# 14chanwa/remotesensingProject

Measured on AMD Instinct MI355X. Metric: Mpixel*disparity-hypotheses/s, higher is better.
Workload: dtype f32

## Files before the change

include/rslf_hip.h:

```cpp
#ifndef RSLF_HIP_H
#define RSLF_HIP_H

#include <stddef.h>
#include <stdint.h>

#ifdef __cplusplus
extern "C" {
#endif

#define RSLF_ABI_VERSION 6

typedef enum rslf_status {
    RSLF_OK = 0,
    RSLF_ERR_INVALID_ARG = -1,
    RSLF_ERR_UNSUPPORTED = -2,
    RSLF_ERR_HIP = -3,
    RSLF_ERR_NO_DEVICE = -4,
    RSLF_ERR_ALLOC = -5,
    RSLF_ERR_INTERNAL = -6
} rslf_status;

typedef struct rslf_params {
    float edge_score_threshold;
    float line_score_threshold;
// ... 327 lines not shown
int rslf_render_fit(rslf_ctx* ctx, const float* d_plane, int rows, int cols, size_t row_stride, const uint8_t* d_valid, int mode,
                    double* h_min, double* h_max);
int rslf_render_fit_many(rslf_ctx* ctx, const float* d_planes, int n_planes, size_t plane_stride, int rows, int cols, size_t row_stride,
                         const uint8_t* d_valid, int mode, double* h_minmax);
int rslf_render_planes(rslf_ctx* ctx, const float* d_planes, int n_planes, size_t plane_stride, int rows, int cols, size_t row_stride,
                       double min, double max, int formula, const uint8_t* lut_bgr, const uint8_t* d_valid, int mask_mode,
                       const rslf_volume* vol, int slice_kind, int index, float shadow_level, uint8_t* d_bgr_out);
int rslf_render_planes_each(rslf_ctx* ctx, const float* d_planes, int n_planes, size_t plane_stride, int rows, int cols, size_t row_stride,
                            const double* h_minmax, int formula, const uint8_t* lut_bgr, const uint8_t* d_valid, int mask_mode,
                            const rslf_volume* vol, int slice_kind, int index, float shadow_level, uint8_t* d_bgr_out);
int rslf_render_planes_host(rslf_ctx* ctx, const float* h_planes, int n_planes, size_t plane_stride, int rows, int cols, size_t row_stride,
                            const uint8_t* h_valid, int fit_mode, int fit_plane, int fit_masked, int formula, const uint8_t* lut_bgr,
                            int mask_mode, const rslf_volume* vol, int slice_kind, int index, float shadow_level, uint8_t* h_bgr_out,
                            double* h_minmax);
int rslf_render_epi_lines(rslf_ctx* ctx, const float* d_depth_vu, const uint8_t* d_mask_vu, int V, int S, int U, int s_hat, int v_first,
                          int n_rows, const uint8_t* lut_bgr, uint8_t* d_bgr_out);
int rslf_render_epi_lines_host(rslf_ctx* ctx, const float* h_depth_vu, const uint8_t* h_mask_vu, int V, int S, int U, int s_hat, int v_first,
                               int n_rows, const uint8_t* lut_bgr, uint8_t* h_bgr_out);
int rslf_render_centre_index(int n, int* index);
int rslf_render_scaled_row(int v, int dim_v, int dim_v_orig, int* row);

int rslf_last_scan_kernel_ms(rslf_ctx* ctx, float* ms);
int rslf_scan_time_total_ms(rslf_ctx* ctx, float* ms, int* launches);

#ifdef __cplusplus
}
#endif
#endif
```

remotesensingproject_amd/_lib.py:

```python
from __future__ import annotations

import ctypes as C
import os

from . import build as _build

_LIB = None

ABI_VERSION = 6

SYMBOLS = [
    "rslf_abi_version", "rslf_status_string", "rslf_last_error", "rslf_device_count", "rslf_default_params",
    "rslf_ctx_create", "rslf_ctx_destroy", "rslf_ctx_set_stream", "rslf_ctx_synchronize", "rslf_ctx_set_debug", "rslf_debug_inject",
    "rslf_multi_create", "rslf_multi_destroy", "rslf_multi_device_count", "rslf_multi_set_chunk_rows", "rslf_multi_peer_access",
    "rslf_multi_depth1d_pile_f32", "rslf_multi_depth1d_pile_u8", "rslf_multi_depth1d_pile_f32_dev",
    "rslf_multi_depth2d_run_f32", "rslf_multi_depth2d_run_u8", "rslf_multi_fine_to_coarse_run_host",
    "rslf_volume_create", "rslf_volume_destroy", "rslf_volume_describe",
    "rslf_volume_upload_epis_f32", "rslf_volume_upload_epis_u8",
    "rslf_volume_upload_images_f32", "rslf_volume_upload_images_u8", "rslf_volume_pack_device_f32",
    "rslf_edge_confidence_pile", "rslf_depth_epi_pile", "rslf_selective_median",
    "rslf_depth1d_pile_run", "rslf_depth1d_pile_run_host", "rslf_last_scan_kernel_ms", "rslf_scan_time_total_ms",
    "rslf_edge_confidence_2d", "rslf_depth_epi_2d", "rslf_depth2d_run",
    "rslf_sweep_begin", "rslf_sweep_visit_scan", "rslf_sweep_visit_finish", "rslf_sweep_end",
    "rslf_depth_epi_scan", "rslf_depth1d_run",
    "rslf_f2c_level_dims", "rslf_downsample_epis_f32", "rslf_downsample_epis_u8", "rslf_device_max_f32", "rslf_f2c_tighten_bounds", "rslf_f2c_fuse",
    "rslf_depth2d_run_host", "rslf_fine_to_coarse_run_host", "rslf_kernel_columns_pile", "rslf_volume_upload_images_xf_f32", "rslf_volume_upload_images_xf_u8",
    "rslf_volume_upload_epis_u16", "rslf_volume_upload_images_u16", "rslf_volume_upload_images_xf_u16", "rslf_downsample_epis_u16",
    "rslf_multi_depth1d_pile_u16", "rslf_multi_depth2d_run_u16", "rslf_fine_to_coarse_run_host_u16",
    "rslf_multi_fine_to_coarse_run_host_u16",
    "rslf_render_fit", "rslf_render_planes", "rslf_render_epi_lines", "rslf_render_centre_index", "rslf_render_scaled_row",
    "rslf_render_fit_many", "rslf_render_planes_each", "rslf_render_planes_host", "rslf_render_epi_lines_host",
    "rslf_line_confidence_pile", "rslf_sweep_line_confidence", "rslf_depth_epi_2d_lc", "rslf_depth2d_run_lc", "rslf_depth2d_run_host_lc",
    "rslf_f2c_pyramid_dims", "rslf_fine_to_coarse_run_host_lc", "rslf_fine_to_coarse_run_host_u16_lc",
    "rslf_f2c_run_host", "rslf_f2c_run_destroy", "rslf_f2c_run_describe", "rslf_f2c_run_copy", "rslf_f2c_run_volume",
    "rslf_f2c_run_render_depth_maps", "rslf_f2c_run_render_depth_maps_host", "rslf_f2c_run_render_depth_pyr",
    "rslf_f2c_run_render_depth_pyr_host", "rslf_f2c_run_render_epi_pyr", "rslf_f2c_run_render_epi_pyr_host",
    "rslf_depth_epi_scores", "rslf_depth_epi_scores_host",
]


class RslfParams(C.Structure):

    _fields_ = [
        ("edge_score_threshold", C.c_float),
# ... 108 lines not shown
    L.rslf_volume_upload_images_f32.argtypes = [vp, C.POINTER(vp), C.c_size_t, cf, C.POINTER(cf)]
    L.rslf_volume_upload_images_u8.argtypes = [vp, C.POINTER(vp), C.c_size_t]
    L.rslf_volume_upload_images_xf_f32.argtypes = [vp, C.POINTER(vp), C.c_size_t, cf, C.POINTER(cf), ci, ci]
    L.rslf_volume_upload_images_xf_u8.argtypes = [vp, C.POINTER(vp), C.c_size_t, ci, ci]
    L.rslf_volume_upload_epis_u16.argtypes = L.rslf_volume_upload_epis_f32.argtypes
    L.rslf_volume_upload_images_u16.argtypes = L.rslf_volume_upload_images_f32.argtypes
    L.rslf_volume_upload_images_xf_u16.argtypes = L.rslf_volume_upload_images_xf_f32.argtypes
    L.rslf_volume_pack_device_f32.argtypes = [vp, vp, cf, C.POINTER(cf)]
    L.rslf_edge_confidence_pile.argtypes = [vp, vp, ci, C.POINTER(RslfParams), vp, vp]
    L.rslf_depth_epi_pile.argtypes = [vp, vp, vp, vp, cf, cf, ci, ci, vp, vp, vp, vp, vp, C.POINTER(RslfParams),
                                      vp, vp, vp, vp, C.POINTER(RslfStats)]
    L.rslf_selective_median.argtypes = [vp, vp, vp, vp, ci, ci, vp, cf]
    L.rslf_depth_epi_scan.argtypes = [vp, vp, vp, vp, cf, cf, ci, ci, vp, vp, vp, vp, vp, C.POINTER(RslfParams),
                                      vp, vp, vp, C.POINTER(RslfStats)]
    L.rslf_depth_epi_scores.argtypes = [vp, vp, vp, vp, cf, cf, ci, ci, C.POINTER(RslfParams), vp, ci, ci, vp, C.POINTER(RslfStats)]
    L.rslf_depth_epi_scores_host.argtypes = L.rslf_depth_epi_scores.argtypes
    L.rslf_depth1d_run.argtypes = [vp, vp, cf, cf, ci, ci, C.POINTER(RslfParams), vp, vp, vp, vp, vp, vp, vp,
                                   C.POINTER(RslfStats)]
    L.rslf_depth1d_pile_run.argtypes = [vp, vp, cf, cf, ci, ci, C.POINTER(RslfParams), vp, vp, vp, vp, vp, vp, vp, vp,
                                        C.POINTER(RslfStats)]
    L.rslf_depth1d_pile_run_host.argtypes = L.rslf_depth1d_pile_run.argtypes
    L.rslf_last_scan_kernel_ms.argtypes = [vp, C.POINTER(cf)]
    L.rslf_scan_time_total_ms.argtypes = [vp, C.POINTER(cf), C.POINTER(ci)]
    L.rslf_sweep_begin.argtypes = [vp, vp, vp, vp, ci, ci, ci]
    L.rslf_sweep_visit_scan.argtypes = [vp, vp, vp, vp, cf, cf, ci, ci, vp, vp, vp, vp, vp, C.POINTER(RslfParams)]
    L.rslf_sweep_visit_finish.argtypes = [vp, vp, ci, vp, vp, vp, vp, C.POINTER(RslfParams)]
    L.rslf_sweep_end.argtypes = [vp, ci, ci, C.POINTER(RslfStats)]
    L.rslf_multi_create.argtypes = [C.POINTER(ci), ci, C.POINTER(vp)]
    L.rslf_multi_destroy.argtypes = [vp]
    L.rslf_multi_device_count.argtypes = [vp]
    L.rslf_multi_set_chunk_rows.argtypes = [vp, ci]
    L.rslf_multi_peer_access.argtypes = [vp, ci, ci]
    L.rslf_debug_inject.argtypes = [C.c_char_p, ci]
    L.rslf_multi_depth1d_pile_f32.argtypes = [vp, C.POINTER(vp), C.c_size_t, ci, ci, ci, ci, cf, cf, cf, ci, ci, C.POINTER(RslfParams),
                                              vp, vp, vp, vp, vp, vp, vp, vp, C.POINTER(RslfStats), C.POINTER(cf)]
    L.rslf_multi_depth1d_pile_f32_dev.argtypes = [vp, C.POINTER(vp), C.c_size_t, ci, ci, ci, ci, cf, cf, cf, ci, ci, C.POINTER(RslfParams), ci,
                                                  vp, vp, vp, vp, vp, vp, vp, vp, C.POINTER(RslfStats), C.POINTER(cf)]
    L.rslf_multi_depth1d_pile_u8.argtypes = [vp, C.POINTER(vp), C.c_size_t, ci, ci, ci, ci, cf, cf, ci, ci, C.POINTER(RslfParams),
                                             vp, vp, vp, vp, vp, vp, vp, vp, C.POINTER(RslfStats)]
    L.rslf_multi_depth2d_run_f32.argtypes = [vp, C.POINTER(vp), C.c_size_t, ci, ci, ci, ci, cf, cf, cf, ci, C.POINTER(RslfParams),
                                             vp, vp, vp, vp, vp, vp, C.POINTER(RslfStats), C.POINTER(cf)]
    L.rslf_multi_depth1d_pile_u16.argtypes = L.rslf_multi_depth1d_pile_f32.argtypes
    L.rslf_multi_depth2d_run_u16.argtypes = L.rslf_multi_depth2d_run_f32.argtypes
    L.rslf_multi_depth2d_run_u8.argtypes = [vp, C.POINTER(vp), C.c_size_t, ci, ci, ci, ci, cf, cf, ci, C.POINTER(RslfParams),
                                            vp, vp, vp, vp, vp, vp, C.POINTER(RslfStats)]
    L.rslf_multi_fine_to_coarse_run_host.argtypes = [vp, C.POINTER(vp), ci, ci, ci, ci, ci, C.c_size_t, cf, cf, ci, cf, C.POINTER(RslfParams),
# ... 68 lines not shown
```

remotesensingproject_amd/csrc/k2_reg.hpp:

```cpp
#pragma once

#include "k2_scan.hpp"
#include "k2_taps.hpp"

namespace rslf {

#ifndef RSLF_REG_GB104
#define RSLF_REG_GB104 8
#endif
constexpr int gather_batch(int c) { return c == 1 ? 8 : 4; }
constexpr int kPadSlack = 16;

template <int SPAD, int C, bool PK, bool KONLY>
__device__ __forceinline__ void mean_shift_pass(const float (&R)[PK ? 1 : C][PK ? 1 : SPAD], const f2 (&R2)[PK ? C : 1][PK ? SPAD / 2 : 1],
                                                int S, float kq, const float (&rbar)[C], float (&A)[C], float& B)
{
    static_assert(!KONLY || (C == 1 && !PK), "the K-only pass is written for the scalar one-channel blocks");
    if constexpr (PK) {
        f2 rb2[C];
        const f2 kq2 = {kq, kq};
#pragma unroll
        for (int c = 0; c < C; c++)
            rb2[c] = f2{rbar[c], rbar[c]};
        constexpr int kBlk = (C == 1) ? 8 : 4;
// ... 456 lines not shown
#ifndef RSLF_REG_BEST_LDS
#define RSLF_REG_BEST_LDS 1
#endif
constexpr bool scan_reg_best_in_lds(int spad, int c)
{
    if (!RSLF_REG_BEST_LDS)
        return false;
    if (c == 1)
        return spad == 16 || spad == 40 || spad == 48 || (spad >= 80 && spad <= 88) || (spad >= 104 && spad <= 144);
    return spad == 24 || spad == 40;
}

constexpr bool scan_reg_packed_math(int spad, int c) { return scan_reg_waves(spad, c) == 1; }

constexpr bool scan_reg_trim(int spad, int c)
{
    return c == 1 && !scan_reg_packed_math(spad, c) && spad != 48 && !(spad >= 80 && spad <= 88) && !(spad > 112 && spad <= 144);
}
#ifndef RSLF_TAP_TABLE
#define RSLF_TAP_TABLE 1
#endif
constexpr bool scan_reg_tap_table(int spad, int c) { return RSLF_TAP_TABLE && c == 1 && spad == 104 && scan_reg_trim(spad, c); }

template <int SPAD, int C>
using ScanRegRbarFix = std::conditional_t<scan_reg_trim(SPAD, C), LastPassRbar<C>, NoRbarFix>;

template <int SPAD, int C, class BestT>
__device__ __forceinline__ void scan_reg_rows(const ScanArgs& a, int v, int u, int d0, int d1, BestT& best, float* otab)
{
    constexpr bool PK = scan_reg_packed_math(SPAD, C);
    constexpr bool kTaps = scan_reg_tap_table(SPAD, C);
    if (a.dmin_vu) {
        scan_reg_body<SPAD, C, true, false, PK, 0, BestT, false, scan_reg_trim(SPAD, C)>(a, v, u, d0, d1, best, otab);
        return;
    }
    const float max_ds = (float)max(a.s_hat, a.vol.S - 1 - a.s_hat);
    const float range = a.dmax - a.dmin, denom = (float)(a.dim_d - 1);
    const float uf = (float)u, Um1 = (float)(a.vol.U - 1);
    auto interior = [&](int d) -> bool {
        const float reach = max_ds * fabsf(hypothesis(a.dmin, range, denom, d)) * fabsf(a.k.slope) + 2.0f;
        return __all((uf - reach >= 0.0f) && (uf + reach <= Um1));
    };
    int d = d0;
    while (d < d1) {
        const bool in = interior(d);
        int e = d + 1;
        while (e < d1 && interior(e) == in)
            e++;
        if (in)
            scan_reg_body<SPAD, C, false, true, PK, 0, BestT, false, scan_reg_trim(SPAD, C), kTaps>(a, v, u, d, e, best, otab);
        else
            scan_reg_body<SPAD, C, true, true, PK, 0, BestT, false, scan_reg_trim(SPAD, C)>(a, v, u, d, e, best, otab);
        d = e;
    }
}

template <int SPAD, int C>
__global__ __launch_bounds__(64 * kScanWaves) __attribute__((amdgpu_waves_per_eu(scan_reg_waves(SPAD, C), scan_reg_waves(SPAD, C))))
void k2_scan_reg(ScanArgs a)
{
    __shared__ __attribute__((aligned(16))) float s_otab[kScanWaves][SPAD * (scan_reg_tap_table(SPAD, C) ? 4 : 1)];
// ... 72 lines not shown
```

remotesensingproject_amd/csrc/k2_scan.hpp:

```cpp
#pragma once

#include <type_traits>

#include "rslf_device.hpp"

namespace rslf {

constexpr int kScanWaves = 4;
#ifndef RSLF_XCD_ROW_INTERLEAVE
#define RSLF_XCD_ROW_INTERLEAVE 1
#endif

struct ScanArgs {
    VolView vol;
    const int* list;
    const int* count;
    const float* dmin_vu;
    const float* dmax_vu;
    float dmin, dmax;
    int dim_d, s_hat;
    ScanConsts k;
    float* Ce;
    uint8_t* Ce_mask;
    float* Cd;
    float* depth;
    float* rbar;
    int32_t* idx;
    float* score;
    int tile_w;
    int tiles_per_row;
    int logical_blocks;
    int per_xcd;
    int groups;
    struct Partial* partial;
    int* ticket;
    int v0;
    int packed;
    const int* packed_n;
    int packed_adapt;
    int stream_park;
    int stream_wave_floats;
    float stream_frac_max;
    int px_waves;
    const int* rowbase;
    int row_min;
    int tap_table;
};

struct Partial {
    float score, D;
    int d;
    float rbar[3];
    double sum;
};

template <int C>
struct Best {
    float score;
    int d;
    float D;
    float rbar[C];
    double sum;
    __device__ __forceinline__ void init()
    {
        score = -1.0f;
        d = 0;
        D = 0.0f;
#pragma unroll
        for (int c = 0; c < C; c++)
            rbar[c] = 0.0f;
// ... 549 lines not shown
```

remotesensingproject_amd/csrc/k2_taps.hpp:

```cpp
#pragma once

#include <math.h>
#include <stdint.h>
#include <string.h>

#if defined(__HIPCC__)
#define RSLF_TAPS_FN __host__ __device__ __forceinline__
#else
#define RSLF_TAPS_FN inline
#endif

namespace rslf {

struct TapEntry {
    int byteoff;
    float t, omt;
    bool fast;
};

RSLF_TAPS_FN uint32_t tap_float_bits(float x)
{
#if defined(__HIP_DEVICE_COMPILE__)
    return __float_as_uint(x);
#else
// ... 20 lines not shown
#else
    return (int)floorf(x);
#endif
}

RSLF_TAPS_FN TapEntry tap_entry(float off, int u_first, int u_last, int U, int C, int row_floats)
{
    const float uf = (float)u_first, ul = (float)u_last;
    const float x_first = off + uf;
    const float x_last = off + ul;
    TapEntry e;
    e.t = tap_fract(x_first);
    const int i0 = tap_floor(x_first);
    e.omt = 1.0f - e.t;
    e.byteoff = (int)((unsigned)(i0 * C + row_floats) << 2);
    const bool inside = x_first > 0.0f && x_last <= (float)(U - 1);
    const bool binade = ((tap_float_bits(x_first) ^ tap_float_bits(x_last)) >> 23) == 0;
    const float back = x_last - ul;
    const bool exact = back == off;
    e.fast = inside && (binade || exact);
    return e;
}

}
```

remotesensingproject_amd/csrc/rslf_core.hip:

```cpp
#include "rslf_internal.hpp"

#include <algorithm>
#include <cmath>

#include "k0_pack.hpp"

using namespace rslf;


namespace rslf {

char* last_error_buffer()
{
    static thread_local char g_err[512] = "";
    return g_err;
}

static std::atomic<int> g_inject[kInjectSites];

bool inject_hit(InjectSite site)
{
    std::atomic<int>& c = g_inject[site];
    int v = c.load(std::memory_order_relaxed);
    while (v > 0)
// ... 194 lines not shown
    ctx->stream = (hipStream_t)hip_stream;
    return RSLF_OK;
}
RSLF_API_CATCH

extern "C" int rslf_ctx_set_debug(rslf_ctx* ctx, const char* key, int value) RSLF_API_TRY
{
    if (!ctx || !key)
        return fail(RSLF_ERR_INVALID_ARG, "ctx/key is NULL");
    if (strcmp(key, "force_scan") == 0 && value >= 0 && value <= 2)
        ctx->force_scan = value;
    else if (strcmp(key, "force_groups") == 0 && value >= 0 && value <= 64)
        ctx->force_groups = value;
    else if (strcmp(key, "force_packed") == 0 && value >= -1 && value <= 1)
        ctx->force_packed = value;
    else if (strcmp(key, "px") == 0 && value >= -1 && value <= 1)
        ctx->px_mode = value;
    else if (strcmp(key, "stream_share") == 0 && value >= 0 && value <= 2)
        ctx->stream_share = value;
    else if (strcmp(key, "row_split") == 0 && value >= 0 && value <= 65536)
        ctx->row_split = value;
    else if (strcmp(key, "tap_table") == 0 && (value == 0 || value == 1))
        ctx->tap_table = value;
    else if (strcmp(key, "claim_skip") == 0 && (value == 0 || value == 1))
        ctx->claim_skip = value;
    else if (strcmp(key, "time_all") == 0 && (value == 0 || value == 1)) {
        ctx->time_all = value;
        ctx->ev_used = 0;
    } else if (strcmp(key, "stream_groups") == 0 && value >= 0 && value <= 64)
        ctx->stream_groups = value;
    else if (strcmp(key, "stream_lds_kib") == 0 && value >= 16 && value <= 152) {
        ctx->stream_lds_bytes = (size_t)value << 10;
    } else if (strcmp(key, "staging_kib") == 0 && value >= 0 && value <= 262144)
        ctx->staging_kib = value;
    else
        return fail(RSLF_ERR_INVALID_ARG, "rslf_ctx_set_debug: unknown key or value out of range: %s = %d", key, value);
    return RSLF_OK;
}
RSLF_API_CATCH

extern "C" int rslf_ctx_synchronize(rslf_ctx* ctx) RSLF_API_TRY
{
    if (!ctx)
        return fail(RSLF_ERR_INVALID_ARG, "ctx is NULL");
    HIP_TRY(hipSetDevice(ctx->device));
    HIP_TRY(hipStreamSynchronize(ctx->stream));
// ... 484 lines not shown
```

remotesensingproject_amd/csrc/rslf_internal.hpp:

```cpp
#pragma once

#include "../../include/rslf_hip.h"

#include <hip/hip_runtime.h>

#include <atomic>
#include <cstdarg>
#include <cstdio>
#include <cstring>
#include <exception>
#include <functional>
#include <memory>
#include <new>
#include <string>
#include <thread>
#include <vector>

#include "rslf_device.hpp"
#include "rslf_plan.hpp"
#include "rslf_scratch.hpp"


namespace rslf {

// ... 112 lines not shown
enum SharedBuf {
    kSharedLevel = 0,
    kSharedTable,
    kSharedLeft,
    kSharedRight,
    kSharedStagePlanes,
    kSharedStageMask,
    kSharedStageOut,
    kSharedBufs
};

struct Scratch {
    DeviceBuf total;
    DeviceBuf minmax;
    DeviceBuf list;
    DeviceBuf depth_tmp;
    DeviceBuf count;
    DeviceBuf rowbase;
    DeviceBuf partial;
    DeviceBuf staging;
    DeviceBuf scan_partial;
    DeviceBuf scan_ticket;
    DeviceBuf max_partial;
    DeviceBuf winner;
    DeviceBuf sweep_mask;
    DeviceBuf dirty;
    DeviceBuf remain;
    DeviceBuf filtered;
    DeviceBuf lc_columns;
    DeviceBuf lc_argmax;
    DeviceBuf shared[kSharedBufs];

    static constexpr size_t kMaxPartials = 2048;
    unsigned long long* pixel_total() const { return total.as<unsigned long long>(); }
    int* packed_len() const { return reinterpret_cast<int*>(pixel_total() + 1); }
    uint8_t* morph_tmp() const { return depth_tmp.as<uint8_t>(); }
};

struct SweepState {
    bool open = false;
    bool keep_total = false;
    bool first = true;
    bool scanned = false;
    bool listed = false;
    int expect = -1;
    uint8_t* mask_run = nullptr;
    int lc_mode = RSLF_LINE_CONF_OFF;
    float* lc_Cl_svu = nullptr;
    float* lc_K_vsu = nullptr;
    int32_t* lc_idx_vu = nullptr;
    const float* lc_Ce_svu = nullptr;
    const float* lc_dmin_vu = nullptr;
    const float* lc_dmax_vu = nullptr;
    float lc_dmin = 0.0f, lc_dmax = 0.0f;
    int lc_dim_d = 0;
    ScanConsts lc_consts = {};
};

}

struct rslf_ctx {
    int device = 0;
    hipStream_t stream = nullptr;
    rslf::Scratch scratch;
    rslf::SweepState sweep;
    hipEvent_t ev0 = nullptr, ev1 = nullptr;
    bool ev_valid = false;
    int time_all = 0;
    std::vector<hipEvent_t> ev_pool;
    size_t ev_used = 0;
    int last_spad = 0;
    int last_kernel = 0;
    int num_cus = 0;
    int force_scan = 0;
    int force_groups = 0;
    int force_packed = -1;
    int px_mode = -1;
    int stream_groups = 0;
    int stream_share = 1;
    size_t stream_lds_bytes = rslf::plan::kStreamLdsBytes;
    int row_split = 1;
    int tap_table = 1;
    int claim_skip = 1;
    int staging_kib = 0;
};

struct rslf_volume {
    rslf_ctx* ctx = nullptr;
    int device = 0;
    int V = 0, S = 0, U = 0, C = 0, pitch = 0;
    float* base = nullptr;
    size_t bytes = 0;
    float min_value = 0.0f, max_value = 0.0f;
    bool filled = false;
};

struct rslf_multi {
    struct Dev {
        rslf_ctx* ctx = nullptr;
        hipStream_t s_up = nullptr, s_comp = nullptr, s_down = nullptr;
        hipEvent_t done[2] = {nullptr, nullptr};
        rslf_volume* vol[2] = {nullptr, nullptr};
        rslf::DeviceBuf planes[2];
        rslf::PinnedBuf pin[2];
        rslf::DeviceBuf arena;
// ... 143 lines not shown
```

remotesensingproject_amd/csrc/rslf_pile.hip:

```cpp
#include "rslf_internal.hpp"

#include <algorithm>
#include <cmath>

#include "k1_edge.hpp"
#include "k2_scan.hpp"
#include "k2_reg.hpp"
#include "k2_stream.hpp"
#include "k3_median.hpp"

using namespace rslf;

static_assert(sizeof(Partial) == plan::kPartialRecordBytes, "rslf_plan.hpp sizes the record scratch");
static_assert(kScanWaves == plan::kScanWavesPerTile, "rslf_plan.hpp shares the hypotheses out over this many waves");


extern "C" int rslf_edge_confidence_pile(rslf_ctx* ctx, const rslf_volume* vol, int s, const rslf_params* p,
                                         float* d_Ce_vu, uint8_t* d_Ce_mask_vu) RSLF_API_TRY
{
    if (!ctx || !vol || !d_Ce_vu || !d_Ce_mask_vu)
        return fail(RSLF_ERR_INVALID_ARG, "NULL argument");
    int rc = check_params(p);
    if (rc)
        return rc;
    if (s < 0 || s >= vol->S)
        return fail(RSLF_ERR_INVALID_ARG, "s=%d outside [0,%d)", s, vol->S);
    if (!vol->filled)
        return fail(RSLF_ERR_INVALID_ARG, "volume has not been filled");
    HIP_TRY(hipSetDevice(ctx->device));
    EdgeConsts ec;
    ec.filter_size = p->edge_confidence_filter_size;
    ec.cut_shadows = p->cut_shadows;
    ec.shadow_level = p->shadow_level;
    ec.edge_thr = p->edge_score_threshold;
    const dim3 grid((vol->U + 255) / 256, vol->V);
    if (vol->C == 1)
        hipLaunchKernelGGL(k1_edge_confidence<1>, grid, dim3(256), 0, ctx->stream, view_of(vol), s, ec, d_Ce_vu, d_Ce_mask_vu);
// ... 121 lines not shown
{
    const int spad = plan::pick_spad(S, C);
    return plan::ScanKernelFacts{spad ? scan_reg_waves(spad, C) : 0, stream_resident_for(S, C), stream_px_resident_for(S, C)};
}

static plan::ScanRequest scan_request(const rslf_ctx* ctx, int V, int U, int S, int C, int dim_d, bool in_range, bool linear,
                                      bool pixel_ranges, const ScanInputs& in)
{
    plan::ScanRequest rq = {};
    rq.V = V, rq.U = U, rq.S = S, rq.C = C, rq.dim_d = dim_d;
    rq.num_cus = ctx->num_cus;
    rq.ctx_groups = in.groups;
    rq.ctx_packed = in.packed;
    rq.precompacted = in.lists;
    rq.force_groups = ctx->force_groups;
    rq.force_packed = ctx->force_packed;
    rq.px_mode = ctx->px_mode;
    rq.stream_groups = ctx->stream_groups;
    rq.stream_share = ctx->stream_share;
    rq.stream_lds_bytes = ctx->stream_lds_bytes;
    rq.tap_table = ctx->tap_table;
    const bool dense_uniform = !pixel_ranges && !in.packed && ctx->force_packed != 1 && in.lists != ScanInputs::kPackedList;
    plan::choose_scan_kernel(&rq, in_range, linear, ctx->force_scan, dense_uniform, kernel_facts(S, C));
    return rq;
}

int rslf::scan_presize(rslf_ctx* ctx, int S, int U, int C, int dim_d, const rslf_params* p, const int* rows, int n_rows)
{
    const plan::ScanKernelFacts f = kernel_facts(S, C);
    int max_rows = 0;
    size_t recs = 0, tickets = 0;
    for (int i = 0; i < n_rows; i++) {
        max_rows = std::max(max_rows, rows[i]);
        ScanInputs in;
        if (p && plan::fuse_k1_compaction(p->edge_confidence_opening_size, ctx->force_packed, (size_t)rows[i] * U))
            in.lists = ScanInputs::kRowLists;
        const plan::ScanRequest rq = scan_request(ctx, rows[i], U, S, C, dim_d, true, !p || p->interpolation == RSLF_INTERP_LINEAR, false, in);
        const plan::ScanPlan sp = plan::plan_scan(rq, f.nres, f.nres_px);
        recs = std::max(recs, sp.records);
        tickets = std::max(tickets, sp.tickets);
    }
    if (max_rows < 1)
        return RSLF_OK;
    HIP_TRY(hipSetDevice(ctx->device));
    bool tickets_fresh = false;
    int rc = ensure_plane_scratch(ctx, max_rows, U);
// ... 32 lines not shown

ScanInputs rslf::scan_defaults(const rslf_ctx* ctx)
{
    ScanInputs in;
    in.zero_total = !ctx->sweep.keep_total;
    in.timed = !ctx->sweep.open || ctx->sweep.first;
    return in;
}

static int check_scan_args(const rslf_volume* vol, const float* d_dmin_vu, const float* d_dmax_vu, int dim_d, int s_hat,
                           const rslf_params* p)
{
    int rc = check_params(p);
    if (rc)
        return rc;
    if ((d_dmin_vu == nullptr) != (d_dmax_vu == nullptr))
        return fail(RSLF_ERR_INVALID_ARG, "d_dmin_vu and d_dmax_vu must both be given or both be NULL");
    if (dim_d < 2)
        return fail(RSLF_ERR_INVALID_ARG, "dim_d=%d: the hypothesis grid divides by dim_d-1 (core.hpp:548)", dim_d);
    if (s_hat < 0 || s_hat >= vol->S)
        return fail(RSLF_ERR_INVALID_ARG, "s_hat=%d outside [0,%d)", s_hat, vol->S);
    if (!vol->filled)
        return fail(RSLF_ERR_INVALID_ARG, "volume has not been filled");
    return RSLF_OK;
}

static void apply_plan(ScanArgs& a, const plan::ScanPlan& p, const rslf_ctx* ctx)
{
    a.groups = p.groups;
    a.tile_w = p.tile_w;
    a.tiles_per_row = p.tiles_per_row;
    a.packed = p.packed ? 1 : 0;
    a.packed_adapt = p.packed_adapt ? 1 : 0;
    a.px_waves = p.px_waves;
    a.tap_table = p.tap_table;
    a.stream_park = p.stream_park;
    a.stream_wave_floats = p.stream_wave_floats;
    a.partial = p.groups > 1 ? ctx->scratch.scan_partial.as<Partial>() : nullptr;
    a.ticket = p.groups > 1 ? ctx->scratch.scan_ticket.as<int>() : nullptr;
}

static int enqueue_scan(const plan::ScanPlan& p, const ScanArgs& a, unsigned grid_x, size_t stream_lds_bytes, hipStream_t st)
{
    const dim3 grid(grid_x), block(64 * kScanWaves);
    const int C = a.vol.C;
    hipError_t attr = hipSuccess;
// ... 98 lines not shown
    a.list = sc.list.as<int>();
    a.count = sc.count.as<int>();
    a.dmin_vu = d_dmin_vu;
    a.dmax_vu = d_dmax_vu;
    a.dmin = dmin;
    a.dmax = dmax;
    a.dim_d = dim_d;
    a.s_hat = s_hat;
    a.k = make_scan_consts(p);
    a.Ce = d_Ce_vu;
    a.Ce_mask = d_Ce_mask_vu;
    a.Cd = d_Cd_vu;
    a.depth = d_depth_vu;
    a.rbar = d_rbar_vu;
    a.idx = d_idx_vu;
    a.score = d_score_vu;
    a.stream_frac_max = plan::stream_frac_max(vol->U);
    a.packed_n = packed_n;
    a.row_min = row_min;
    ScanArgs ar = a;
    apply_plan(a, sp, ctx);
    apply_plan(ar, spr, ctx);
    ar.rowbase = sc.rowbase.as<int>();
    ctx->last_spad = sp.spad;
    ctx->last_kernel = sp.kind;
    HIP_TRY(hipGetLastError());

    const bool pooled = ctx->time_all && ctx->ev_used + 2 <= ((size_t)1 << 16);
    while (pooled && ctx->ev_pool.size() < ctx->ev_used + 2) {
        hipEvent_t e = nullptr;
        HIP_TRY(hipEventCreate(&e));
        ctx->ev_pool.push_back(e);
    }
    auto enqueue_all = [&]() -> int {
        if (pooled)
            HIP_TRY(hipEventRecord(ctx->ev_pool[ctx->ev_used - 2], st));
        if (in.timed)
            HIP_TRY(hipEventRecord(ctx->ev0, st));
        for (const plan::ScanLaunch& l : row_launches) {
            ar.v0 = l.v0, ar.logical_blocks = l.logical_blocks, ar.per_xcd = l.per_xcd;
            if (int e = enqueue_scan(spr, ar, l.grid, ctx->stream_lds_bytes, st))
                return e;
        }
        for (const plan::ScanLaunch& l : launches) {
            a.v0 = l.v0, a.logical_blocks = l.logical_blocks, a.per_xcd = l.per_xcd;
            if (int e = enqueue_scan(sp, a, l.grid, ctx->stream_lds_bytes, st))
// ... 212 lines not shown
}
RSLF_API_CATCH

extern "C" int rslf_scan_time_total_ms(rslf_ctx* ctx, float* ms, int* launches) RSLF_API_TRY
{
    if (!ctx || !ms)
        return fail(RSLF_ERR_INVALID_ARG, "NULL argument");
    HIP_TRY(hipSetDevice(ctx->device));
    double sum = 0.0;
    for (size_t i = 0; i + 1 < ctx->ev_used; i += 2) {
        float t = 0.0f;
        HIP_TRY(hipEventSynchronize(ctx->ev_pool[i + 1]));
        HIP_TRY(hipEventElapsedTime(&t, ctx->ev_pool[i], ctx->ev_pool[i + 1]));
        sum += (double)t;
    }
    *ms = (float)sum;
    if (launches)
        *launches = (int)(ctx->ev_used / 2);
    ctx->ev_used = 0;
    return RSLF_OK;
}
RSLF_API_CATCH

extern "C" int rslf_last_scan_kernel_ms(rslf_ctx* ctx, float* ms) RSLF_API_TRY
{
    if (!ctx || !ms)
        return fail(RSLF_ERR_INVALID_ARG, "NULL argument");
    if (!ctx->ev_valid)
        return fail(RSLF_ERR_INVALID_ARG, "no scan kernel has been launched on this context");
    HIP_TRY(hipSetDevice(ctx->device));
    HIP_TRY(hipEventSynchronize(ctx->ev1));
    HIP_TRY(hipEventElapsedTime(ms, ctx->ev0, ctx->ev1));
    return RSLF_OK;
}
RSLF_API_CATCH
```

remotesensingproject_amd/csrc/rslf_plan.hpp:

```cpp
#pragma once

#include <stddef.h>
#include <stdint.h>

#include <string.h>

#include <algorithm>
#include <cmath>
#include <vector>

#include "../../include/rslf_hip.h"

namespace rslf {

struct MorphElement {
    int k;
    unsigned rows[31];
};

namespace plan {


constexpr int kScanWavesPerTile = 4;
constexpr size_t kPartialRecordBytes = 32;
// ... 556 lines not shown
            best = w;
        }
    }
    return best_use >= 0.6 ? best : 0;
}

struct ScanRequest {
    int V, U, S, C, dim_d;
    int spad;
    bool use_stream;
    bool use_chip;
    int chip_wave_floats;
    int reg_waves;
    int num_cus;
    int ctx_groups;
    bool ctx_packed;
    int precompacted;
    int force_groups;
    int force_packed;
    int px_mode;
    int stream_groups;
    int stream_share;
    size_t stream_lds_bytes;
    int tap_table;
};

struct ScanPlan {
    int kind;
    int spad;
    int groups;
    bool packed;
    bool packed_adapt;
    int px_waves;
    int tap_table;
    int tile_w;
    int tiles_per_row;
    int rows_per_launch;
    size_t records;
    size_t tickets;
    int stream_nres;
    int stream_park;
    int stream_wave_floats;
    size_t lds_bytes;
};

inline int stream_resident_hi(int C, int nres_1ch, int nres_rgb) { return C == 1 ? nres_1ch : nres_rgb; }

struct ScanKernelFacts {
    int reg_waves;
    int nres;
    int nres_px;
};

inline bool scan_range_ok(float min_value, float max_value) { return min_value >= 0.0f && max_value <= 1.0e6f; }

inline void choose_scan_kernel(ScanRequest* r, bool in_range, bool linear, int force_scan, bool dense_uniform, const ScanKernelFacts& f)
{
// ... 61 lines not shown
    if (packed && (r.spad || r.use_stream) && !r.use_chip && r.px_mode != 0) {
        px_w = px_waves(r.dim_d);
        if (px_w == 0 && r.px_mode == 1)
            px_w = 1;
    }
    if (px_w && r.use_stream && nres_px >= 0)
        nres = nres_px;
    p.stream_nres = r.use_stream ? nres : 0;
    const int park_early = r.use_stream ? stream_park_for(r.S, r.C, nres, r.stream_lds_bytes) : 0;
    const bool share = r.use_chip ? r.stream_share != 0
                                  : r.use_stream && (r.stream_share == 2 || (r.stream_share == 1 && stream_shares_taps(r.S, nres, park_early)));
    p.tile_w = (share && !packed) ? 63 : 64;
    p.tiles_per_row = p.tile_w == 63 ? std::max(1, (r.U + 61) / 63) : (r.U + p.tile_w - 1) / p.tile_w;
    p.packed_adapt = packed && !r.use_stream && !r.use_chip;
    p.rows_per_launch = r.V;
    if (groups > 1 && !packed) {
        const size_t per_row = (size_t)p.tiles_per_row * groups * 64 * kPartialRecordBytes;
        p.rows_per_launch = (int)std::min<size_t>((size_t)r.V, std::max<size_t>(1, kPartialBudget / per_row));
    }
    if (packed && (r.use_stream || r.use_chip))
        while (groups > 1 && ((n + 63) / 64) * groups * 64 * kPartialRecordBytes > kPartialBudget)
            groups /= 2;
    p.px_waves = px_w;
    p.tap_table = (r.spad && !packed && r.tap_table) ? 1 : 0;
    p.spad = r.spad;
    p.kind = r.spad ? (px_w ? RSLF_SCAN_REG_PX : RSLF_SCAN_REG)
             : r.use_chip ? RSLF_SCAN_CHIP
             : r.use_stream ? (px_w ? RSLF_SCAN_STREAM_PX : RSLF_SCAN_STREAM) : RSLF_SCAN_GENERIC;
    if (px_w) {
        groups = 1;
        p.packed_adapt = false;
    }
    p.groups = groups;
    p.packed = packed;
    p.records = 0;
    p.tickets = 0;
    if (groups > 1) {
        const size_t tiles_all = (n + 63) / 64;
        const size_t tiles_max = !packed ? (size_t)p.rows_per_launch * p.tiles_per_row
                                         : p.packed_adapt ? std::min<size_t>(tiles_all, kPackedItemTarget / 2) : tiles_all;
        p.records = (packed && p.packed_adapt) ? std::min<size_t>(tiles_all * groups, kPackedItemTarget) * 64 : tiles_max * groups * 64;
        p.tickets = tiles_max;
    }
    p.stream_park = 0;
    p.stream_wave_floats = 0;
    p.lds_bytes = 0;
    if (r.use_stream) {
// ... 261 lines not shown
```

remotesensingproject_amd/depth.py:

```python
from __future__ import annotations

import atexit
import copy
import ctypes as C
import sys
from dataclasses import dataclass
from typing import Optional, Sequence

import numpy as np
import torch

from . import _lib
from ._lib import RslfParams, RslfStats, RslfVolumeDesc, check


class Interpolation1DLinear:
    mode = 0


class Interpolation1DNearestNeighbour:

    def __init__(self, as_built: bool = False):
        self.mode = 2 if as_built else 1

# ... 43 lines not shown
        raise ValueError("%s: par_line_confidence_mode=%d is not built here (one-device Depth2DComputer only)"
                         % (who, int(parameters.par_line_confidence_mode)))


class Context:

    def __init__(self, device: int | torch.device | None = None):
        if device is None:
            device = torch.cuda.current_device()
        self.device = torch.device("cuda", device) if isinstance(device, int) else torch.device(device)
        h = C.c_void_p()
        check(_lib.lib().rslf_ctx_create(self.device.index or 0, C.byref(h)), "rslf_ctx_create")
        self._h = h
        self.use_current_stream()

    def use_current_stream(self) -> None:
        s = torch.cuda.current_stream(self.device).cuda_stream
        check(_lib.lib().rslf_ctx_set_stream(self._h, C.c_void_p(s)), "rslf_ctx_set_stream")

    def synchronize(self) -> None:
        check(_lib.lib().rslf_ctx_synchronize(self._h), "rslf_ctx_synchronize")

    _DEBUG_DEFAULTS = dict(force_scan=0, force_groups=0, force_packed=-1, px=-1, stream_share=1, stream_groups=0, stream_lds_kib=80,
                           claim_skip=1, time_all=0, row_split=1, staging_kib=0, tap_table=1)
    _FORCE_SCAN = {None: 0, "auto": 0, "generic": 1, "stream": 2}

    def set_debug(self, **hooks) -> None:
        for k, v in hooks.items():
            if k == "force_scan" and not isinstance(v, int):
                v = self._FORCE_SCAN[v or None]
            check(_lib.lib().rslf_ctx_set_debug(self._h, k.encode(), int(v)), "rslf_ctx_set_debug(%s)" % k)

    def reset_debug(self) -> None:
        self.set_debug(**self._DEBUG_DEFAULTS)

    def last_scan_kernel_ms(self) -> float:
        ms = C.c_float()
        check(_lib.lib().rslf_last_scan_kernel_ms(self._h, C.byref(ms)), "rslf_last_scan_kernel_ms")
        return float(ms.value)

    def scan_time_total_ms(self) -> tuple[float, int]:
        ms, n = C.c_float(), C.c_int()
        check(_lib.lib().rslf_scan_time_total_ms(self._h, C.byref(ms), C.byref(n)), "rslf_scan_time_total_ms")
        return float(ms.value), int(n.value)

    def close(self) -> None:
        if getattr(self, "_h", None) and not sys.is_finalizing():
            _lib.lib().rslf_ctx_destroy(self._h)
        self._h = None

    def __del__(self):
        try:
            self.close()
        except Exception:
            pass


_DEFAULT_CTX: dict[int, Context] = {}


@atexit.register
def _drop_default_contexts() -> None:
# ... 1104 lines not shown
```

Before: 8353.

## Precompute per-hypothesis row tap offsets and weights for scalar-load register scan

```diff
diff --git a/include/rslf_hip.h b/include/rslf_hip.h
--- a/include/rslf_hip.h
+++ b/include/rslf_hip.h
@@ -373,6 +373,7 @@
 
 int rslf_last_scan_kernel_ms(rslf_ctx* ctx, float* ms);
 int rslf_scan_time_total_ms(rslf_ctx* ctx, float* ms, int* launches);
+int rslf_last_scan_row_exact(rslf_ctx* ctx, int* attached, int* exact_hypotheses);
 
 #ifdef __cplusplus
 }
diff --git a/remotesensingproject_amd/_lib.py b/remotesensingproject_amd/_lib.py
--- a/remotesensingproject_amd/_lib.py
+++ b/remotesensingproject_amd/_lib.py
@@ -19,7 +19,7 @@
     "rslf_volume_upload_epis_f32", "rslf_volume_upload_epis_u8",
     "rslf_volume_upload_images_f32", "rslf_volume_upload_images_u8", "rslf_volume_pack_device_f32",
     "rslf_edge_confidence_pile", "rslf_depth_epi_pile", "rslf_selective_median",
-    "rslf_depth1d_pile_run", "rslf_depth1d_pile_run_host", "rslf_last_scan_kernel_ms", "rslf_scan_time_total_ms",
+    "rslf_depth1d_pile_run", "rslf_depth1d_pile_run_host", "rslf_last_scan_kernel_ms", "rslf_scan_time_total_ms", "rslf_last_scan_row_exact",
     "rslf_edge_confidence_2d", "rslf_depth_epi_2d", "rslf_depth2d_run",
     "rslf_sweep_begin", "rslf_sweep_visit_scan", "rslf_sweep_visit_finish", "rslf_sweep_end",
     "rslf_depth_epi_scan", "rslf_depth1d_run",
@@ -174,6 +174,7 @@
     L.rslf_depth1d_pile_run_host.argtypes = L.rslf_depth1d_pile_run.argtypes
     L.rslf_last_scan_kernel_ms.argtypes = [vp, C.POINTER(cf)]
     L.rslf_scan_time_total_ms.argtypes = [vp, C.POINTER(cf), C.POINTER(ci)]
+    L.rslf_last_scan_row_exact.argtypes = [vp, C.POINTER(ci), C.POINTER(ci)]
     L.rslf_sweep_begin.argtypes = [vp, vp, vp, vp, ci, ci, ci]
     L.rslf_sweep_visit_scan.argtypes = [vp, vp, vp, vp, cf, cf, ci, ci, vp, vp, vp, vp, vp, C.POINTER(RslfParams)]
     L.rslf_sweep_visit_finish.argtypes = [vp, vp, ci, vp, vp, vp, vp, C.POINTER(RslfParams)]
diff --git a/remotesensingproject_amd/csrc/k2_reg.hpp b/remotesensingproject_amd/csrc/k2_reg.hpp
--- a/remotesensingproject_amd/csrc/k2_reg.hpp
+++ b/remotesensingproject_amd/csrc/k2_reg.hpp
@@ -502,6 +502,102 @@
 #endif
 constexpr bool scan_reg_tap_table(int spad, int c) { return RSLF_TAP_TABLE && c == 1 && spad == 104 && scan_reg_trim(spad, c); }
 
+#ifndef RSLF_SCALAR_TAPS
+#define RSLF_SCALAR_TAPS 1
+#endif
+#ifndef RSLF_SCALAR_GB
+#define RSLF_SCALAR_GB 13
+#endif
+constexpr bool scan_reg_scalar_taps(int spad, int c) { return RSLF_SCALAR_TAPS && scan_reg_tap_table(spad, c); }
+
+template <int SPAD, class BestT>
+__device__ __forceinline__ void scan_reg_body_scalar(const ScanArgs& a, int v, int u, int d0, int d1, BestT& best)
+{
+    constexpr int C = 1, BATCH = RSLF_SCALAR_GB, ROUNDS = SPAD / BATCH;
+    static_assert(SPAD % BATCH == 0, "whole rounds");
+    static_assert(!scan_reg_packed_math(SPAD, 1) && scan_reg_trim(SPAD, 1), "the passes below are the scalar TRIM ones of the other forms");
+    typedef const __attribute__((address_space(4))) long long* OffPtr;
+    typedef const __attribute__((address_space(4))) f2* WeightPtr;
+    typedef const __attribute__((address_space(4))) float* FloatPtr;
+    const VolView& vol = a.vol;
+    const float* epi = vol.row(v, 0);
+    const int S = vol.S;
+    const float kq = a.k.k1;
+    const unsigned ubytes = (unsigned)u << 2;
+    const float centre = epi[(long long)a.s_hat * vol.stride_s + u];
+    const f2 R2[1][1] = {{f2{0.0f, 0.0f}}};
+
+#pragma unroll 1
+    for (int d = d0; d < d1; d++) {
+        const float Dd = ((FloatPtr)a.rx_D)[d];
+        const OffPtr toff = (OffPtr)a.rx_off + (long long)d * SPAD;
+        const WeightPtr tw = (WeightPtr)a.rx_w + (long long)d * SPAD;
+        float R[C][SPAD];
+        long long cur[BATCH], nxt[BATCH];
+#pragma unroll
+        for (int j = 0; j < BATCH; j++)
+            cur[j] = toff[j];
+#pragma unroll
+        for (int g = 0; g < ROUNDS; g++) {
+            float e0[BATCH], e1[BATCH];
+            f2 w[BATCH];
+            unsigned ub = ubytes;
+            asm volatile("" : "+v"(ub));
+#pragma unroll
+            for (int j = 0; j < BATCH; j++) {
+                typedef const __attribute__((address_space(1))) char* GlobalBytes;
+                typedef const __attribute__((address_space(1))) float* GlobalFloats;
+                const unsigned long long sum = (unsigned long long)epi + (unsigned long long)cur[j];
+                unsigned lo = (unsigned)sum;
+                asm volatile("" : "+s"(lo));
+                const unsigned long long row = (sum & 0xFFFFFFFF00000000ull) | lo;
+                const GlobalFloats p = (GlobalFloats)((GlobalBytes)row + ub);
+                e0[j] = p[0];
+                e1[j] = p[1];
+            }
+#pragma unroll
+            for (int j = 0; j < BATCH; j++)
+                w[j] = tw[g * BATCH + j];
+            if (g + 1 < ROUNDS) {
+#pragma unroll
+                for (int j = 0; j < BATCH; j++)
+                    nxt[j] = toff[(g + 1) * BATCH + j];
+            }
+#pragma unroll
+            for (int j = 0; j < BATCH; j++) {
+                const float m0 = w[j].y * e0[j];
+                const float m1 = w[j].x * e1[j];
+                R[0][g * BATCH + j] = m0 + m1;
+            }
+#pragma unroll
+            for (int j = 0; j < BATCH; j++)
+                asm volatile("" : "+v"(R[0][g * BATCH + j]));
+#pragma unroll
+            for (int j = 0; j < BATCH; j++)
+                cur[j] = nxt[j];
+        }
+
+        float rbar[C] = {centre};
+        float B = 0.0f;
+#pragma unroll 1
+        for (int it = 0; it < a.k.n_iter; it++) {
+            float A[C] = {0.0f};
+            B = 0.0f;
+            if (it == a.k.n_iter - 1) {
+                mean_shift_pass<SPAD, C, false, true>(R, R2, S, kq, rbar, A, B);
+                break;
+            }
+            mean_shift_pass<SPAD, C, false, false>(R, R2, S, kq, rbar, A, B);
+            const float qd = (B != 0.0f) ? (A[0] / B) : 0.0f;
+            rbar[0] = (qd > 0.0f) ? qd : 0.0f;
+        }
+        const float cardf = (float)S;
+        float sc = (S != 0) ? (B / cardf) : 0.0f;
+        sc = (sc > 0.0f) ? sc : 0.0f;
+        best.offer(sc, d, Dd, rbar);
+    }
+}
+
 template <int SPAD, int C>
 using ScanRegRbarFix = std::conditional_t<scan_reg_trim(SPAD, C), LastPassRbar<C>, NoRbarFix>;
 
@@ -517,6 +613,32 @@
     const float max_ds = (float)max(a.s_hat, a.vol.S - 1 - a.s_hat);
     const float range = a.dmax - a.dmin, denom = (float)(a.dim_d - 1);
     const float uf = (float)u, Um1 = (float)(a.vol.U - 1);
+    if constexpr (scan_reg_scalar_taps(SPAD, C)) {
+        typedef const __attribute__((address_space(4))) float* FloatPtr;
+        typedef const __attribute__((address_space(4))) int* IntPtr;
+        const bool rx = a.rx_off != nullptr;
+        auto form = [&](int d) -> int {
+            const float Dd = rx ? ((FloatPtr)a.rx_D)[d] : hypothesis(a.dmin, range, denom, d);
+            const float reach = max_ds * fabsf(Dd) * fabsf(a.k.slope) + 2.0f;
+            const bool in = __all((uf - reach >= 0.0f) && (uf + reach <= Um1));
+            return !in ? 0 : (rx && ((IntPtr)a.rx_exact)[d]) ? 2 : 1;
+        };
+        int d = d0;
+        while (d < d1) {
+            const int f = form(d);
+            int e = d + 1;
+            while (e < d1 && form(e) == f)
+                e++;
+            if (f == 2)
+                scan_reg_body_scalar<SPAD>(a, v, u, d, e, best);
+            else if (f == 1)
+                scan_reg_body<SPAD, C, false, true, PK, 0, BestT, false, scan_reg_trim(SPAD, C), kTaps>(a, v, u, d, e, best, otab);
+            else
+                scan_reg_body<SPAD, C, true, true, PK, 0, BestT, false, scan_reg_trim(SPAD, C)>(a, v, u, d, e, best, otab);
+            d = e;
+        }
+        return;
+    }
     auto interior = [&](int d) -> bool {
         const float reach = max_ds * fabsf(hypothesis(a.dmin, range, denom, d)) * fabsf(a.k.slope) + 2.0f;
         return __all((uf - reach >= 0.0f) && (uf + reach <= Um1));
diff --git a/remotesensingproject_amd/csrc/k2_scan.hpp b/remotesensingproject_amd/csrc/k2_scan.hpp
--- a/remotesensingproject_amd/csrc/k2_scan.hpp
+++ b/remotesensingproject_amd/csrc/k2_scan.hpp
@@ -45,7 +45,12 @@
     const int* rowbase;
     int row_min;
     int tap_table;
+    const long long* rx_off;
+    const float* rx_w;
+    const float* rx_D;
+    const int* rx_exact;
 };
+
 
 struct Partial {
     float score, D;
diff --git a/remotesensingproject_amd/csrc/k2_taps.hpp b/remotesensingproject_amd/csrc/k2_taps.hpp
--- a/remotesensingproject_amd/csrc/k2_taps.hpp
+++ b/remotesensingproject_amd/csrc/k2_taps.hpp
@@ -66,4 +66,28 @@
     return e;
 }
 
+struct RowExactEntry {
+    int byteoff;
+    float t, omt;
+    bool exact;
+};
+
+RSLF_TAPS_FN RowExactEntry row_exact_entry(float off, int U, int C, int row_floats)
+{
+    const float ul = (float)(U - 1);
+    const float x_last = off + ul;
+    const float back = x_last - ul;
+    RowExactEntry e;
+    const bool sane = x_last >= 1.0f && x_last < 8388608.0f;
+    const float xs = sane ? x_last : 1.0f;
+    e.t = tap_fract(xs);
+    const int i_last = tap_floor(xs);
+    e.omt = 1.0f - e.t;
+    const long long floats = (long long)(i_last - (U - 1)) * C + row_floats;
+    e.byteoff = (int)((unsigned)floats << 2);
+    const bool fits = floats >= -(1LL << 28) && floats < (1LL << 28);
+    e.exact = sane && fits && back == off;
+    return e;
 }
+
+}
diff --git a/remotesensingproject_amd/csrc/rslf_core.hip b/remotesensingproject_amd/csrc/rslf_core.hip
--- a/remotesensingproject_amd/csrc/rslf_core.hip
+++ b/remotesensingproject_amd/csrc/rslf_core.hip
@@ -240,6 +240,8 @@
         ctx->row_split = value;
     else if (strcmp(key, "tap_table") == 0 && (value == 0 || value == 1))
         ctx->tap_table = value;
+    else if (strcmp(key, "scalar_taps") == 0 && (value == 0 || value == 1))
+        ctx->scalar_taps = value;
     else if (strcmp(key, "claim_skip") == 0 && (value == 0 || value == 1))
         ctx->claim_skip = value;
     else if (strcmp(key, "time_all") == 0 && (value == 0 || value == 1)) {
diff --git a/remotesensingproject_amd/csrc/rslf_internal.hpp b/remotesensingproject_amd/csrc/rslf_internal.hpp
--- a/remotesensingproject_amd/csrc/rslf_internal.hpp
+++ b/remotesensingproject_amd/csrc/rslf_internal.hpp
@@ -158,6 +158,7 @@
     DeviceBuf scan_partial;
     DeviceBuf scan_ticket;
     DeviceBuf max_partial;
+    DeviceBuf row_exact;
     DeviceBuf winner;
     DeviceBuf sweep_mask;
     DeviceBuf dirty;
@@ -171,6 +172,22 @@
     unsigned long long* pixel_total() const { return total.as<unsigned long long>(); }
     int* packed_len() const { return reinterpret_cast<int*>(pixel_total() + 1); }
     uint8_t* morph_tmp() const { return depth_tmp.as<uint8_t>(); }
+};
+
+constexpr int row_exact_slots(int spad, int C) { return (C == 1 && spad == 104) ? spad : 0; }
+constexpr size_t row_exact_bytes(int dim_d, int slots) { return (size_t)dim_d * ((size_t)slots * 16 + 8); }
+
+struct RowExactKey {
+    float dmin = 0.0f, dmax = 0.0f, slope = 0.0f;
+    int dim_d = 0, s_hat = 0, S = 0, U = 0, C = 0, slots = 0;
+    long long stride_s = 0;
+    const void* queued_on = nullptr;
+    bool same(const RowExactKey& o) const
+    {
+        return memcmp(&dmin, &o.dmin, sizeof(float)) == 0 && memcmp(&dmax, &o.dmax, sizeof(float)) == 0 &&
+               memcmp(&slope, &o.slope, sizeof(float)) == 0 && dim_d == o.dim_d && s_hat == o.s_hat && S == o.S && U == o.U && C == o.C &&
+               slots == o.slots && stride_s == o.stride_s && queued_on == o.queued_on;
+    }
 };
 
 struct SweepState {
@@ -217,6 +234,9 @@
     size_t stream_lds_bytes = rslf::plan::kStreamLdsBytes;
     int row_split = 1;
     int tap_table = 1;
+    int scalar_taps = 1;
+    rslf::RowExactKey row_exact_key;
+    bool last_row_exact = false;
     int claim_skip = 1;
     int staging_kib = 0;
 };
diff --git a/remotesensingproject_amd/csrc/rslf_pile.hip b/remotesensingproject_amd/csrc/rslf_pile.hip
--- a/remotesensingproject_amd/csrc/rslf_pile.hip
+++ b/remotesensingproject_amd/csrc/rslf_pile.hip
@@ -13,6 +13,8 @@
 
 static_assert(sizeof(Partial) == plan::kPartialRecordBytes, "rslf_plan.hpp sizes the record scratch");
 static_assert(kScanWaves == plan::kScanWavesPerTile, "rslf_plan.hpp shares the hypotheses out over this many waves");
+static_assert(!RSLF_SCALAR_TAPS || !RSLF_TAP_TABLE || (scan_reg_scalar_taps(104, 1) && row_exact_slots(104, 1) == 104),
+              "rslf_internal.hpp names the kernel that has the scalar-tap form");
 
 
 extern "C" int rslf_edge_confidence_pile(rslf_ctx* ctx, const rslf_volume* vol, int s, const rslf_params* p,
@@ -180,6 +182,7 @@
     rq.tap_table = ctx->tap_table;
     const bool dense_uniform = !pixel_ranges && !in.packed && ctx->force_packed != 1 && in.lists != ScanInputs::kPackedList;
     plan::choose_scan_kernel(&rq, in_range, linear, ctx->force_scan, dense_uniform, kernel_facts(S, C));
+    rq.scalar_taps = (ctx->scalar_taps && !pixel_ranges && row_exact_slots(rq.spad, C)) ? 1 : 0;
     return rq;
 }
 
@@ -258,6 +261,68 @@
         return fail(RSLF_ERR_INVALID_ARG, "s_hat=%d outside [0,%d)", s_hat, vol->S);
     if (!vol->filled)
         return fail(RSLF_ERR_INVALID_ARG, "volume has not been filled");
+    return RSLF_OK;
+}
+
+__global__ __launch_bounds__(128) void k2_fill_row_exact(float dmin, float dmax, int dim_d, float slope, int s_hat, int S, int slots, int U,
+                                                         int C, int stride_s, long long* __restrict__ out_off, f2* __restrict__ out_w,
+                                                         float* __restrict__ out_D, int* __restrict__ out_exact)
+{
+    const int d = blockIdx.x, s = threadIdx.x;
+    const float Dd = hypothesis(dmin, dmax - dmin, (float)(dim_d - 1), d);
+    bool ok = true;
+    if (s < slots) {
+        const int sv = min(s, S - 1);
+        float off = (float)(s_hat - sv) * Dd;
+        off = off * slope;
+        const RowExactEntry e = row_exact_entry(off, U, C, sv * stride_s);
+        const long long bo = (long long)e.byteoff;
+        const f2 w = s < S ? f2{e.t, e.omt} : f2{0.0f, 0.0f};
+        ok = e.exact;
+        out_off[(size_t)d * slots + s] = bo;
+        out_w[(size_t)d * slots + s] = w;
+    }
+    const int all = __syncthreads_and(ok ? 1 : 0);
+    if (s == 0) {
+        out_D[d] = Dd;
+        out_exact[d] = all ? 1 : 0;
+    }
+}
+
+static int attach_row_exact(rslf_ctx* ctx, ScanArgs& a, const plan::ScanPlan& p, hipStream_t st)
+{
+    const bool has_form = p.kind == RSLF_SCAN_REG && !p.packed && a.vol.C == 1 && p.spad == 104 && scan_reg_scalar_taps(104, 1);
+    const int slots = has_form && p.scalar_taps && !a.dmin_vu ? row_exact_slots(p.spad, a.vol.C) : 0;
+    ctx->last_row_exact = false;
+    if (!slots || a.vol.S > slots || a.vol.S <= slots - 16 || slots > 128 || a.vol.stride_s * (long long)slots > INT32_MAX)
+        return RSLF_OK;
+    RowExactKey key;
+    key.dmin = a.dmin, key.dmax = a.dmax, key.slope = a.k.slope;
+    key.dim_d = a.dim_d, key.s_hat = a.s_hat, key.S = a.vol.S, key.U = a.vol.U, key.C = a.vol.C, key.slots = slots;
+    key.stride_s = a.vol.stride_s;
+    key.queued_on = st;
+    const Reserved r = ctx->scratch.row_exact.reserve(row_exact_bytes(a.dim_d, slots));
+    if (r.err) {
+        ctx->row_exact_key = RowExactKey{};
+        HIP_TRY(hip_err(r));
+    }
+    char* base = ctx->scratch.row_exact.as<char>();
+    long long* d_off = reinterpret_cast<long long*>(base);
+    f2* d_w = reinterpret_cast<f2*>(d_off + (size_t)a.dim_d * slots);
+    float* d_D = reinterpret_cast<float*>(d_w + (size_t)a.dim_d * slots);
+    int* d_exact = reinterpret_cast<int*>(d_D + a.dim_d);
+    if (r.fresh || !key.same(ctx->row_exact_key)) {
+        ctx->row_exact_key = RowExactKey{};
+        hipLaunchKernelGGL(k2_fill_row_exact, dim3(a.dim_d), dim3(128), 0, st, a.dmin, a.dmax, a.dim_d, a.k.slope, a.s_hat, a.vol.S, slots,
+                           a.vol.U, a.vol.C, (int)a.vol.stride_s, d_off, d_w, d_D, d_exact);
+        HIP_TRY(hipGetLastError());
+        ctx->row_exact_key = key;
+    }
+    a.rx_off = d_off;
+    a.rx_w = reinterpret_cast<const float*>(d_w);
+    a.rx_D = d_D;
+    a.rx_exact = d_exact;
+    ctx->last_row_exact = true;
     return RSLF_OK;
 }
 
@@ -402,6 +467,9 @@
     apply_plan(a, sp, ctx);
     apply_plan(ar, spr, ctx);
     ar.rowbase = sc.rowbase.as<int>();
+    rc = attach_row_exact(ctx, a, sp, st);
+    if (rc)
+        return rc;
     ctx->last_spad = sp.spad;
     ctx->last_kernel = sp.kind;
     HIP_TRY(hipGetLastError());
@@ -660,6 +728,26 @@
 }
 RSLF_API_CATCH
 
+extern "C" int rslf_last_scan_row_exact(rslf_ctx* ctx, int* attached, int* exact_hypotheses) RSLF_API_TRY
+{
+    if (!ctx || !attached || !exact_hypotheses)
+        return fail(RSLF_ERR_INVALID_ARG, "NULL argument");
+    *attached = ctx->last_row_exact ? 1 : 0;
+    *exact_hypotheses = 0;
+    if (!ctx->last_row_exact)
+        return RSLF_OK;
+    HIP_TRY(hipSetDevice(ctx->device));
+    const RowExactKey& k = ctx->row_exact_key;
+    std::vector<int> flags((size_t)k.dim_d);
+    const char* d_flags = ctx->scratch.row_exact.as<char>() + (size_t)k.dim_d * ((size_t)k.slots * 16 + sizeof(float));
+    HIP_TRY(hipMemcpyAsync(flags.data(), d_flags, flags.size() * sizeof(int), hipMemcpyDeviceToHost, ctx->stream));
+    HIP_TRY(hipStreamSynchronize(ctx->stream));
+    for (int f : flags)
+        *exact_hypotheses += f != 0;
+    return RSLF_OK;
+}
+RSLF_API_CATCH
+
 extern "C" int rslf_last_scan_kernel_ms(rslf_ctx* ctx, float* ms) RSLF_API_TRY
 {
     if (!ctx || !ms)
diff --git a/remotesensingproject_amd/csrc/rslf_plan.hpp b/remotesensingproject_amd/csrc/rslf_plan.hpp
--- a/remotesensingproject_amd/csrc/rslf_plan.hpp
+++ b/remotesensingproject_amd/csrc/rslf_plan.hpp
@@ -602,7 +602,7 @@
     int stream_groups;
     int stream_share;
     size_t stream_lds_bytes;
-    int tap_table;
+    int tap_table, scalar_taps;
 };
 
 struct ScanPlan {
@@ -612,7 +612,7 @@
     bool packed;
     bool packed_adapt;
     int px_waves;
-    int tap_table;
+    int tap_table, scalar_taps;
     int tile_w;
     int tiles_per_row;
     int rows_per_launch;
@@ -720,7 +720,7 @@
         while (groups > 1 && ((n + 63) / 64) * groups * 64 * kPartialRecordBytes > kPartialBudget)
             groups /= 2;
     p.px_waves = px_w;
-    p.tap_table = (r.spad && !packed && r.tap_table) ? 1 : 0;
+    p.tap_table = (r.spad && !packed && r.tap_table) ? 1 : 0, p.scalar_taps = (p.tap_table && r.scalar_taps) ? 1 : 0;
     p.spad = r.spad;
     p.kind = r.spad ? (px_w ? RSLF_SCAN_REG_PX : RSLF_SCAN_REG)
              : r.use_chip ? RSLF_SCAN_CHIP
diff --git a/remotesensingproject_amd/depth.py b/remotesensingproject_amd/depth.py
--- a/remotesensingproject_amd/depth.py
+++ b/remotesensingproject_amd/depth.py
@@ -89,7 +89,7 @@
         check(_lib.lib().rslf_ctx_synchronize(self._h), "rslf_ctx_synchronize")
 
     _DEBUG_DEFAULTS = dict(force_scan=0, force_groups=0, force_packed=-1, px=-1, stream_share=1, stream_groups=0, stream_lds_kib=80,
-                           claim_skip=1, time_all=0, row_split=1, staging_kib=0, tap_table=1)
+                           claim_skip=1, time_all=0, row_split=1, staging_kib=0, tap_table=1, scalar_taps=1)
     _FORCE_SCAN = {None: 0, "auto": 0, "generic": 1, "stream": 2}
 
     def set_debug(self, **hooks) -> None:
@@ -105,6 +105,11 @@
         ms = C.c_float()
         check(_lib.lib().rslf_last_scan_kernel_ms(self._h, C.byref(ms)), "rslf_last_scan_kernel_ms")
         return float(ms.value)
+
+    def last_scan_row_exact(self) -> tuple[bool, int]:
+        a, n = C.c_int(), C.c_int()
+        check(_lib.lib().rslf_last_scan_row_exact(self._h, C.byref(a), C.byref(n)), "rslf_last_scan_row_exact")
+        return bool(a.value), int(n.value)
 
     def scan_time_total_ms(self) -> tuple[float, int]:
         ms, n = C.c_float(), C.c_int()
```

Measured after the change: 8599 (median of 6 runs). 2.9% higher.
